# yjxiong/action-detection

Measured on AMD Instinct MI355X. Metric: proposals/sec (9-seg BNInception SSN fwd+bwd), higher is better.
Workload: dtype f32

## Files before the change

### action-detection_amd/_lib.py

```python
import ctypes
import os
import subprocess
import threading

import torch

_HERE = os.path.dirname(os.path.abspath(__file__))
CSRC = os.path.join(_HERE, "csrc")
LIB_PATH = os.path.join(_HERE, "libssn_hip.so")
SOURCES = ["conv_igemm.hip", "conv_x6.hip", "conv_x6_rect.hip", "conv_wgrad.hip", "conv_wgrad_x6.hip", "elementwise.hip", "bn_train.hip", "frames.hip", "detect.hip", "pool.hip", "stpp.hip", "heads_losses.hip", "conv_pl.hip", "planes_ops.hip", "planes_bn.hip", "wgrad_pl.hip", "tag.hip", "eval.hip", "actionness.hip", "train_step.hip"]

STPP_MAX_PARTS = 24


class SsnStppTable(ctypes.Structure):
    _fields_ = [("n_parts", ctypes.c_int), ("n_seg", ctypes.c_int),
                ("act_lo", ctypes.c_int), ("act_hi", ctypes.c_int),
                ("lo", ctypes.c_int * STPP_MAX_PARTS), ("hi", ctypes.c_int * STPP_MAX_PARTS),
                ("norm", ctypes.c_int * STPP_MAX_PARTS), ("col", ctypes.c_int * STPP_MAX_PARTS)]


_SIGS = {
    "ssn_conv_bn_relu_fwd": "pppppiiiiliiiliiiiipp",
    "ssn_bn_fold": "pppppfppip",
    "ssn_relu_bn_bwd": "pppiiillpp",
    "ssn_conv_dgrad": "pppiiiiliiiliiiiplpiipp",
    "ssn_conv_pack_weights": "ppiiiip",
    "ssn_conv_pack_weights_multi": "ippppppppp",
    "ssn_conv_wgrad": "ppppiiiiliiiliiiplip",
    "ssn_conv_wgrad_x6": "ppppiiiililiiiplippiipp",
    "ssn_wgrad_reduce": "pppiiip",
    "ssn_wgrad_reduce_taps": "pppiiiip",
    "ssn_conv_x6_pack_weights_multi": "ippppppppppppp",
    "ssn_conv_x6_fwd": "pppppiiiiliiiliiiiiippiiipp",
    "ssn_conv_x6_dgrad": "pppiiiiliiiliiiplpiippiipp",
    "ssn_conv_x6_fwd_rect": "pppppiiiiliiiliiiiiiippp",
    "ssn_conv_x6_pack_dgrad_s2": "ppiip",
    "ssn_conv_x6_dgrad_s2": "pppiiiiliiiliplpiippip",
    "ssn_conv_x6_pack_dgrad_rect": "ppiiiip",
    "ssn_conv_x6_pack_rect_multi": "ipppppppp",
    "ssn_conv_x6_dgrad_rect": "pppiiiililiiiiiplpiippp",
    "ssn_conv_wgrad_x6_rect": "ppppiiiililiiiiiplippp",
    "ssn_conv_x6_pack_weights_rect": "ppiiiip",
    "ssn_pool_fwd": "ipppiiiiliiliiipp",
    "ssn_pool_bwd": "ipppiiiiliiliiiiplppp",
    "ssn_avgpool_affine_fwd": "ppppiiiiiliiliiipp",
    "ssn_channel_sum": "ppiiilpup",
    "ssn_tensor_amax": "plpp",
    "ssn_bn_train_stats": "ppppppiiilffpup",
    "ssn_bn_train_apply": "ppppppiiiillpp",
    "ssn_bn_train_bwd": "pppppppppiiiillllpupp",
    "ssn_global_avgpool_fwd": "ppiiilp",
    "ssn_global_avgpool_bwd": "ppiiilipp",
    "ssn_dropout_fwd": "ppplfupp",
    "ssn_dropout_bwd": "ppplfp",
    "ssn_stpp_fwd": "ppppiipp",
    "ssn_stpp_bwd": "ppppiipp",
    "ssn_heads_fwd": "pppppppppppiipp",
    "ssn_heads_bwd": "pppppppppppiippppp",
    "ssn_stpp_reorg": "piippppiiiiipppp",
    "ssn_crop_mean": "ppiiip",
    "ssn_detections": "ppppppppuiiiiidip",
    "ssn_tag_count": "pppiipidppppp",
    "ssn_tag_generate": "ppppiipipippllddppppppppup",
    "ssn_tag_name_proposals": "pppippiidpppp",
    "ssn_eval_count": "ppiipp",
    "ssn_eval_ap": "ppppippiippiippllpppplp",
    "ssn_eval_recall": "ppippiipipp",
    "ssn_actionness_fc": "ppppiiiiiip",
    "ssn_actionness_group": "pppiiiip",
    "ssn_actionness_merge": "pppppiiiiip",
    "ssn_frames_crop_normalize": "ppiiiiiiipppiipipip",
    "ssn_frames_crop_resize_normalize": "ppiiiiiippiipipipup",
    "ssn_reg_denorm": "plffffp",
    "ssn_frame_diff": "ppliiip",
    "ssn_linear_fwd": "ppppiiip",
    "ssn_linear_bwd": "ppppppiiiip",
    "ssn_row_gather": "pppiip",
    "ssn_row_scatter": "pppiiip",
    "ssn_ce_loss_fwd": "ppppiip",
    "ssn_ce_loss_bwd": "pppppiip",
    "ssn_completeness_loss_fwd": "pppppiiiiiifp",
    "ssn_completeness_loss_bwd": "ppppiifp",
    "ssn_cw_smoothl1_fwd": "pppppiip",
    "ssn_total_loss_fwd": "ppiippiiiiiifpppiiffpppppp",
    "ssn_total_loss_bwd": "ppiipiifpiiffpppppppp",
    "ssn_label_select": "pppipipippppp",
    "ssn_param_checksum": "pipppip",
    "ssn_cw_smoothl1_bwd": "ppppiip",
    "ssn_sgd_step": "ppplffffipp",
    "ssn_sgd_step_multi": "ippppppffipp",
    "ssn_bn_fold_multi": "ipppppppppp",
    "ssn_sumsq": "plpipp",
# ... 54 lines not shown
        self.cdll.ssn_abi_version.restype = ctypes.c_int
        self.cdll.ssn_conv_wgrad_workspace_bytes.restype = ctypes.c_long
        self.cdll.ssn_conv_wgrad_workspace_bytes.argtypes = [ctypes.c_int] * 7
        self.cdll.ssn_conv_packed_floats.restype = ctypes.c_long
        self.cdll.ssn_conv_packed_floats.argtypes = [ctypes.c_int] * 4
        self.cdll.ssn_conv_x6_packed_floats.restype = ctypes.c_long
        self.cdll.ssn_conv_x6_packed_floats.argtypes = [ctypes.c_int] * 4
        self.cdll.ssn_conv_x6_dgrad_s2_packed_floats.restype = ctypes.c_long
        self.cdll.ssn_conv_x6_dgrad_s2_packed_floats.argtypes = [ctypes.c_int] * 2
        self.cdll.ssn_conv_x6_packed_floats_rect.restype = ctypes.c_long
        self.cdll.ssn_conv_x6_packed_floats_rect.argtypes = [ctypes.c_int] * 4
        self.cdll.ssn_conv_x6_packed_floats_dgrad_rect.restype = ctypes.c_long
        self.cdll.ssn_conv_x6_packed_floats_dgrad_rect.argtypes = [ctypes.c_int] * 4
        self.cdll.ssn_conv_wgrad_x6_rect_workspace_bytes.restype = ctypes.c_long
        self.cdll.ssn_conv_wgrad_x6_rect_workspace_bytes.argtypes = [ctypes.c_int] * 8
        self.cdll.ssn_conv_wgrad_x6_workspace_bytes.restype = ctypes.c_long
        self.cdll.ssn_conv_wgrad_x6_workspace_bytes.argtypes = [ctypes.c_int] * 7
        self.cdll.ssn_detections_workspace_bytes.restype = ctypes.c_size_t
        self.cdll.ssn_detections_workspace_bytes.argtypes = [ctypes.c_int] * 2
        self.cdll.ssn_tag_workspace_bytes.restype = ctypes.c_size_t
        self.cdll.ssn_tag_workspace_bytes.argtypes = [ctypes.c_long] * 2
        self.cdll.ssn_tag_lds_candidates.restype = ctypes.c_int
        self.cdll.ssn_tag_lds_candidates.argtypes = []
        self.cdll.ssn_eval_workspace_bytes.restype = ctypes.c_size_t
        self.cdll.ssn_eval_workspace_bytes.argtypes = [ctypes.c_long, ctypes.c_long, ctypes.c_int]
        self.cdll.ssn_eval_lds_gt.restype = ctypes.c_int
        self.cdll.ssn_eval_lds_gt.argtypes = []
        self.cdll.ssn_sumsq_multi_workspace_floats.restype = ctypes.c_long
        self.cdll.ssn_sumsq_multi_workspace_floats.argtypes = [ctypes.c_int, ctypes.c_void_p]
        self.cdll.ssn_train_step_launches.restype = ctypes.c_long
        self.cdll.ssn_train_step_launches.argtypes = [ctypes.c_int]
        self.cdll.ssn_conv_pick_tile.restype = ctypes.c_int
        self.cdll.ssn_conv_pick_tile.argtypes = [ctypes.c_int, ctypes.c_long]
        self.cdll.ssn_pl_channel_sum_workspace_bytes.restype = ctypes.c_long
        self.cdll.ssn_pl_channel_sum_workspace_bytes.argtypes = [ctypes.c_int]
        self.cdll.ssn_conv_x6_pack_entry_bytes.restype = ctypes.c_long
        self.cdll.ssn_conv_x6_pack_batch_abort.restype = None
        self.cdll.ssn_pl_bn_train_workspace_bytes.restype = ctypes.c_long
        self.cdll.ssn_pl_bn_train_workspace_bytes.argtypes = [ctypes.c_int]
        self.cdll.ssn_frames_resize_workspace_bytes.restype = ctypes.c_size_t
        self.cdll.ssn_frames_resize_workspace_bytes.argtypes = [ctypes.c_int] * 3
        self.cdll.ssn_conv_wgrad_pl_workspace_bytes.restype = ctypes.c_long
        self.cdll.ssn_conv_wgrad_pl_workspace_bytes.argtypes = [ctypes.c_int] * 8
        self.cdll.ssn_conv_wgrad_pl_group_workspace_bytes.restype = ctypes.c_long
        self.cdll.ssn_conv_wgrad_pl_group_workspace_bytes.argtypes = [ctypes.c_int, ctypes.c_void_p, ctypes.c_void_p, ctypes.c_void_p]
        self.cdll.ssn_conv_wgrad_pl_group_table_bytes.restype = ctypes.c_long
        self.cdll.ssn_conv_wgrad_pl_group_table_bytes.argtypes = [ctypes.c_int]
        self.cdll.ssn_conv_wgrad_pl_group_tuning.restype = None
        self.cdll.ssn_conv_wgrad_pl_group_tuning.argtypes = [ctypes.c_double, ctypes.c_double, ctypes.c_int, ctypes.c_int]
        self._fn = {}
        for name, sig in _SIGS.items():
            fn = getattr(self.cdll, name)
            fn.restype = ctypes.c_int
            fn.argtypes = [_CT[c] for c in sig]
            self._fn[name] = fn

    def call(self, name, *args):
        rc = self._fn[name](*args)
        if rc != 0:
            raise RuntimeError("%s failed (%d): %s" % (name, rc, self.cdll.ssn_last_error().decode()))

    def wgrad_workspace_bytes(self, n, cin, cout, ho, wo, ksize, tile_cfg=-1):
        return int(self.cdll.ssn_conv_wgrad_workspace_bytes(n, cin, cout, ho, wo, ksize, tile_cfg))


_lock = threading.Lock()
_lib = None
_test_lib = None


def _source_stamp(deps, flags):
    import hashlib
    h = hashlib.sha256(" ".join(flags).encode())
    for d in deps:
        h.update(os.path.basename(d).encode())
        with open(d, "rb") as f:
            h.update(f.read())
    return h.hexdigest()


def build(force=False, verbose=False):
    import fcntl
    srcs = [os.path.join(CSRC, s) for s in SOURCES]
    deps = srcs + [os.path.join(CSRC, h) for h in ("ssn_common.h", "conv_epilogue.h", "conv_x6_kernel.h", "planes.h", "conv_pl_epilogue.inc")]
    flags = ["--offload-arch=gfx950", "-O3", "-std=c++17", "-fPIC"]
    stamp_path = LIB_PATH + ".stamp"
    want = _source_stamp(deps, flags)

    def fresh():
        if not os.path.exists(LIB_PATH) or not os.path.exists(stamp_path):
            return False
        with open(stamp_path) as f:
            return f.read().strip() == want

    if not force and fresh():
        return LIB_PATH
    with open(LIB_PATH + ".lock", "w") as lock:
        fcntl.flock(lock, fcntl.LOCK_EX)
        try:
            if not force and fresh():
                return LIB_PATH
            hipcc = os.environ.get("HIPCC", "/opt/rocm/bin/hipcc")
            objs = []
            procs = []
            headers = deps[len(srcs):]
            for s in srcs:
                o = os.path.join(CSRC, os.path.basename(s) + ".o")
                objs.append(o)
                ostamp = _source_stamp([s] + headers, flags)
                try:
                    with open(o + ".stamp") as f:
                        if not force and os.path.exists(o) and f.read().strip() == ostamp:
                            continue
                except OSError:
                    pass
                cmd = [hipcc] + flags + ["-c", s, "-o", o]
                procs.append((cmd, o, ostamp, subprocess.Popen(cmd, stdout=subprocess.PIPE, stderr=subprocess.STDOUT)))
            for cmd, o, ostamp, p in procs:
                out, _ = p.communicate()
                if verbose and out:
                    print(out.decode())
                if p.returncode != 0:
                    raise RuntimeError("hipcc failed: %s\n%s" % (" ".join(cmd), out.decode()))
                with open(o + ".stamp", "w") as f:
                    f.write(ostamp + "\n")
            tmp = LIB_PATH + ".tmp.%d" % os.getpid()
            subprocess.check_call([hipcc, "--offload-arch=gfx950", "-shared", "-fPIC", "-o", tmp] + objs)
            os.replace(tmp, LIB_PATH)
            with open(stamp_path, "w") as f:
                f.write(want + "\n")
        finally:
            fcntl.flock(lock, fcntl.LOCK_UN)
    return LIB_PATH


def get_lib():
    global _lib
    if _test_lib is not None:
        return _test_lib
    if _lib is None:
        with _lock:
            if _lib is None:
                if not os.path.exists(LIB_PATH):
                    raise RuntimeError(
                        "libssn_hip.so is missing (%s). Build it with __graft_entry__.build() / "
                        "action_detection_amd.build(); there is no CPU fallback." % LIB_PATH)
                _lib = SsnLibrary(LIB_PATH)
    return _lib


def use_library_for_testing(lib):
    global _test_lib
    _test_lib = lib


def emulator_active():
    return _test_lib is not None and _test_lib.is_emulator
```

### action-detection_amd/csrc/conv_pl.hip

```cpp
#include "planes.h"

namespace {

using namespace pl;

enum { MODE_FWD = 0, MODE_DGRAD = 1 };

constexpr int APITCH = 16;

struct PlConvArgs {
    const void* x_hi;
    const void* x_lo;
    const uint32_t* ap;
    const float* x_scale;
    const float* y_scale;
    float* y_amax;
    void* y_hi;
    void* y_lo;
    const float* scale;
    const float* shift;
    int N, C, H, W;
    uint32_t x_img_bytes;
    uint32_t x_grp_bytes;
    int M;
    int Ho, Wo;
    uint32_t y_img_bytes, y_grp_bytes;
    int P;
    int kh, kw, stride, pad_h, pad_w;
    int relu, accumulate;
    int raw_from;
    int row_split, row_gap;
    int k_split, k_gap;
    const void* mask_hi;
    const float* mask_scale;
    uint32_t mask_img_bytes;
    int n_ptiles, n_mtiles, ngroups;
    uint32_t x_bytes, a_bytes, y_bytes, mask_bytes;
    int sub_a, sub_b, sub_W;
    uint32_t magic_wp;
    FastDiv div_sp;
    unsigned long long* trace;
    int dbg;
    FastDiv div_hw, div_w, div_mt;
    FastDiv div_tpi;
};

#ifdef PL_ABLATE
#define PL_DBG(bit) (p.dbg & (bit))
#else
#define PL_DBG(bit) 0
#endif

#if defined(__HIP_DEVICE_COMPILE__)
#define PL_DMA_B128(rsrc_, dst_, voff_, soff_) \
    __builtin_amdgcn_raw_ptr_buffer_load_lds(rsrc_, SSN_LDS_PTR(dst_), 16, voff_, soff_, 0, 0)
#else
#define PL_DMA_B128(rsrc_, dst_, voff_, soff_) ((void)(dst_), (void)(voff_), (void)(soff_))
#endif

template <int MODE, int WM, int WN, int TM, int TN>
__global__ __launch_bounds__(256, (TM * TN >= 8) ? 1 : 2) void conv_pl_kernel(PlConvArgs p) {
    constexpr int NW = 4;
    constexpr int NT = 256;
    constexpr int BM = WM * TM * 32;
    constexpr int BN = WN * TN * 32;
    static_assert(WM * WN == 4, "4 waves");
    static_assert(BN % 64 == 0 && BN <= 256, "tile width 64 / 128 / 256 pixels");
    constexpr int SEGS = BN / 64;
    constexpr int A_PIECES = BM / 16;
    constexpr int NA = (A_PIECES + NW - 1) / NW;
    constexpr int A_STAGE = NA * NW * 256;
    constexpr int PK = BN * 4;
    constexpr int B_STAGE = 4 * PK;
    constexpr int STAGE = A_STAGE + B_STAGE;
    constexpr bool ONE_WAVE = (TM * TN >= 8);
    constexpr int NSTAGE = (STAGE * 4 * 4 * (ONE_WAVE ? 1 : 2) <= 163840) ? 4 : 3;
    constexpr int NB = 4 * SEGS / NW;
    constexpr int NLOAD = NA + NB;

    __shared__ __attribute__((aligned(1024))) uint32_t lds[NSTAGE * STAGE];

    const int tid = threadIdx.x;
    const int lane = tid & 63, wave = wave_uniform(tid >> 6);
    const int wm = wave / WN, wn = wave % WN;
    const int li = lane & 31, lh = lane >> 5;

    const uint32_t nblk = (uint32_t)p.n_ptiles * (uint32_t)p.n_mtiles;
    const uint32_t logical = xcd_remap(blockIdx.x, nblk);
    uint32_t ptile, mtile;
    fd_divmod(logical, p.div_mt, ptile, mtile);
    const int m0 = (int)mtile * BM;
    const int p0 = (int)ptile * BN;
    const int KK = p.kh * p.kw;
    unsigned long long tr0 = 0, tr1 = 0, tr2 = 0, trr = 0;
    if (p.trace) {
        tr0 = __builtin_readcyclecounter();
        trr = __builtin_amdgcn_s_memrealtime();
    }

    const int seg = wave % SEGS;
    uint32_t gbase;
    uint32_t gmask = 0;
    {
        const int gp = p0 + seg * 64 + lane;
        const bool gvalid = gp < p.P;
        uint32_t n, hw, ho, wo;
        fd_divmod((uint32_t)(gvalid ? gp : 0), p.div_hw, n, hw);
        fd_divmod(hw, p.div_w, ho, wo);
        const int h0 = (MODE == MODE_FWD) ? (int)ho * p.stride - p.pad_h : (int)ho + p.pad_h;
        const int w0 = (MODE == MODE_FWD) ? (int)wo * p.stride - p.pad_w : (int)wo + p.pad_w;
        int t = 0;
        for (int r = 0; r < p.kh; ++r)
            for (int s = 0; s < p.kw; ++s, ++t) {
                const int hi = (MODE == MODE_FWD) ? h0 + r : h0 - r;
                const int wi = (MODE == MODE_FWD) ? w0 + s : w0 - s;
                if (gvalid && ((unsigned)hi < (unsigned)p.H) && ((unsigned)wi < (unsigned)p.W)) gmask |= 1u << t;
            }
        gbase = n * p.x_img_bytes + (uint32_t)((h0 * p.W + w0) * 16);
        if (PL_DBG(1)) gmask = 0;
    }

    uint32_t aoff[NA];
#pragma unroll
    for (int q = 0; q < NA; ++q) {
        const int f = (q * NW + wave) * 64 + lane;
        aoff[q] = (f < BM * 4 && m0 + f / 4 < p.M && !PL_DBG(2)) ? (uint32_t)(m0 * APITCH) * 4u + (uint32_t)f * 16u : PL_OOB;
    }
    const __amdgpu_buffer_rsrc_t xrsrc[2] = {pl_rsrc(p.x_hi, p.x_bytes), pl_rsrc(p.x_lo, p.x_bytes)};
    const __amdgpu_buffer_rsrc_t arsrc = pl_rsrc(p.ap, p.a_bytes);
    const uint32_t a_step = (uint32_t)(p.M * APITCH) * 4u;
    const int nslab = p.ngroups * KK;
    const bool c_half = (p.C & 8) != 0;

    int pf_g = 0, pf_tap = 0, pf_col = 0;
// ... 359 lines not shown
        __builtin_amdgcn_s_barrier();
        __builtin_amdgcn_sched_barrier(0);
        const int ntap = tap == 8 ? 0 : tap + 1, nhb = tap == 8 ? hb ^ 1 : hb;
        const uint32_t dead = (tap + NSTAGE >= 9) ? tail_dead : 0u;
        auto piece = [&](int k) {
            if (k == 0)
                issue_halo(nx_live, nx_so, hb ^ 1, tap);
            else
                issue_a(s_cur, dead, k - 1);
        };
#pragma unroll
        for (int c = 0; c < 3; ++c)
#pragma unroll
            for (int i = 0; i < TM; ++i)
#pragma unroll
                for (int j = 0; j < TN; ++j) {
                    acc[i][j] = __builtin_amdgcn_mfma_f32_32x32x16_f16(f.af[PA[c]][i], f.bf[PB[c]][j], acc[i][j], 0, 0, 0);
                    const int idx = (c * TM + i) * TN + j;
#pragma unroll
                    for (int k = idx * NREAD / NM; k < (idx + 1) * NREAD / NM; ++k)
                        if (!PL_DBG(4)) read_step(nxt, k, s_n1, nhb, ntap);
                    if ((idx + 1) % EVERY == 0 && (idx + 1) / EVERY <= NLOAD) piece((idx + 1) / EVERY - 1);
                    __builtin_amdgcn_sched_barrier(0);
                }
#pragma unroll
        for (int k = NM / EVERY; k < NLOAD; ++k) piece(k);
        pf_a += a_step;
        const uint32_t o = s_cur;
        s_cur = s_n1;
        s_n1 = s_n2;
        if (NSTAGE == 4) {
            s_n2 = s_n3;
            s_n3 = o;
        } else {
            s_n2 = o;
        }
    };
    auto group = [&](int g, Frags& fa, Frags& fb, int hb) {
        group_begin(g);
#pragma unroll
        for (int tap = 0; tap < 9; ++tap) {
            if (tap & 1)
                slab(fb, fa, tap, hb);
            else
                slab(fa, fb, tap, hb);
        }
    };
    int g = 0;
    for (; g + 1 < p.ngroups; g += 2) {
        group(g, fr0, fr1, 0);
        group(g + 1, fr1, fr0, 1);
    }
    if (g < p.ngroups) group(g, fr0, fr1, 0);
    SSN_WAIT_LGKM0();
    SSN_WAIT_VMCNT(0);

#define PL_PEND (PI ? pl_pend : p.P)
#include "conv_pl_epilogue.inc"
#undef PL_PEND
}
#undef PL_DMA_B128

int g_pl_default_tile = -1;
int g_pl_dbg = 0;
unsigned long long* g_pl_trace = nullptr;

template <int MODE, int WM, int WN, int TM, int TN>
int launch_cfg(PlConvArgs& a, hipStream_t stream) {
    constexpr int BM = WM * TM * 32;
    constexpr int BN = WN * TN * 32;
    a.n_mtiles = (a.M + BM - 1) / BM;
    a.div_mt = make_fastdiv((uint32_t)a.n_mtiles);
    a.n_ptiles = (a.P + BN - 1) / BN;
    const unsigned nblk = (unsigned)a.n_ptiles * (unsigned)a.n_mtiles;
    hipLaunchKernelGGL((conv_pl_kernel<MODE, WM, WN, TM, TN>), dim3(nblk), dim3(256), 0, stream, a);
    SSN_CHECK_LAUNCH("conv_pl");
    return SSN_OK;
}

constexpr int PL_NCFG = 12;
const int kPlBM[PL_NCFG] = {128, 64, 128, 64, 192, 256, 128, 96, 160, 32, 64, 192};
const int kPlBN[PL_NCFG] = {128, 128, 64, 64, 128, 128, 256, 128, 128, 128, 256, 64};

template <int MODE>
int launch_tile(PlConvArgs& a, int cfg, hipStream_t stream) {
    switch (cfg) {
        case 0: return launch_cfg<MODE, 2, 2, 2, 2>(a, stream);
        case 1: return launch_cfg<MODE, 2, 2, 1, 2>(a, stream);
        case 2: return launch_cfg<MODE, 2, 2, 2, 1>(a, stream);
        case 3: return launch_cfg<MODE, 2, 2, 1, 1>(a, stream);
        case 4: return launch_cfg<MODE, 2, 2, 3, 2>(a, stream);
        case 5: return launch_cfg<MODE, 2, 2, 4, 2>(a, stream);
        case 6: return launch_cfg<MODE, 2, 2, 2, 4>(a, stream);
        case 7: return launch_cfg<MODE, 1, 4, 3, 1>(a, stream);
        case 8: return launch_cfg<MODE, 1, 4, 5, 1>(a, stream);
        case 9: return launch_cfg<MODE, 1, 4, 1, 1>(a, stream);
        case 10: return launch_cfg<MODE, 2, 2, 1, 4>(a, stream);
        case 11: return launch_cfg<MODE, 2, 2, 3, 1>(a, stream);
    }
    ssn_set_error("conv_pl: unknown tile config %d", cfg);
    return SSN_ERR_ARG;
}

template <int MODE, int WM, int WN, int TM, int TN, bool PI = false>
int launch_cfg9(PlConvArgs& a, hipStream_t stream) {
    constexpr int BM = WM * TM * 32;
    constexpr int BN = WN * TN * 32;
    a.n_mtiles = (a.M + BM - 1) / BM;
    a.div_mt = make_fastdiv((uint32_t)a.n_mtiles);
    if (PI) {
        const int tpi = (a.H * a.W + BN - 1) / BN;
        a.div_tpi = make_fastdiv((uint32_t)tpi);
        a.n_ptiles = a.N * tpi;
    } else {
        a.div_tpi = make_fastdiv(1u);
        a.n_ptiles = (a.P + BN - 1) / BN;
    }
    const unsigned nblk = (unsigned)a.n_ptiles * (unsigned)a.n_mtiles;
    hipLaunchKernelGGL((conv_pl9_kernel<MODE, WM, WN, TM, TN, PI>), dim3(nblk), dim3(256), 0, stream, a);
    SSN_CHECK_LAUNCH("conv_pl9");
    return SSN_OK;
}
bool halo_tile_pi(int cfg) { return cfg == 0 || cfg == 1 || cfg == 4 || cfg == 7 || cfg == 8 || cfg == 9; }
template <int MODE>
int launch_tile9_pi(PlConvArgs& a, int cfg, hipStream_t stream) {
    switch (cfg) {
        case 0: return launch_cfg9<MODE, 2, 2, 2, 2, true>(a, stream);
        case 1: return launch_cfg9<MODE, 2, 2, 1, 2, true>(a, stream);
        case 4: return launch_cfg9<MODE, 2, 2, 3, 2, true>(a, stream);
        case 7: return launch_cfg9<MODE, 1, 4, 3, 1, true>(a, stream);
        case 8: return launch_cfg9<MODE, 1, 4, 5, 1, true>(a, stream);
        case 9: return launch_cfg9<MODE, 1, 4, 1, 1, true>(a, stream);
    }
    ssn_set_error("conv_pl9: tile config %d has no per-image haloed variant", cfg);
    return SSN_ERR_ARG;
}
bool halo_fits_pi(int H, int W, int bn, int hs) {
    const int Wp = W + 2;
    auto slot = [&](int q) { return (q / W + 1) * Wp + (q % W) + 1; };
    for (int p0 = 0; p0 < H * W; p0 += bn) {
        const int p1 = p0 + bn - 1 < H * W - 1 ? p0 + bn - 1 : H * W - 1;
        if (slot(p1) - slot(p0) + 2 * (Wp + 1) + 1 > hs) return false;
    }
    return true;
}
bool halo_tile(int cfg) { return cfg == 0 || cfg == 1 || cfg == 2 || cfg == 3 || cfg == 4 || cfg == 7 || cfg == 8 || cfg == 9 || cfg == 11; }
template <int MODE>
int launch_tile9(PlConvArgs& a, int cfg, hipStream_t stream) {
    switch (cfg) {
        case 0: return launch_cfg9<MODE, 2, 2, 2, 2>(a, stream);
        case 1: return launch_cfg9<MODE, 2, 2, 1, 2>(a, stream);
        case 2: return launch_cfg9<MODE, 2, 2, 2, 1>(a, stream);
        case 3: return launch_cfg9<MODE, 2, 2, 1, 1>(a, stream);
        case 4: return launch_cfg9<MODE, 2, 2, 3, 2>(a, stream);
        case 7: return launch_cfg9<MODE, 1, 4, 3, 1>(a, stream);
        case 8: return launch_cfg9<MODE, 1, 4, 5, 1>(a, stream);
        case 9: return launch_cfg9<MODE, 1, 4, 1, 1>(a, stream);
        case 11: return launch_cfg9<MODE, 2, 2, 3, 1>(a, stream);
    }
    ssn_set_error("conv_pl9: tile config %d has no haloed variant", cfg);
    return SSN_ERR_ARG;
}
bool halo_fits(int N, int H, int W, int bn, int hs) {
    const long P = (long)N * H * W;
    const int Wp = W + 2, SP = (H + 2) * Wp;
    auto slot = [&](long pp) { return (pp / (H * W)) * SP + ((pp % (H * W)) / W + 1) * Wp + (pp % W) + 1; };
    for (long t = 0; t * bn < P; ++t) {
        const long p0 = t * bn, p1 = (p0 + bn - 1 < P - 1) ? p0 + bn - 1 : P - 1;
// ... 19 lines not shown
    }
    if (cfg >= PL_HALO_BASE) {
        cfg -= PL_HALO_BASE;
        if (halo_layer && cfg < PL_NCFG && halo_tile(cfg) && halo_fits(a.N, a.H, a.W, kPlBN[cfg], kPlBN[cfg] == 128 ? 320 : 192)) {
            a.magic_wp = (uint32_t)((0x100000000ull + (unsigned)(a.W + 2) - 1) / (unsigned)(a.W + 2));
            a.div_sp = make_fastdiv((uint32_t)((a.H + 2) * (a.W + 2)));
            return launch_tile9<MODE>(a, cfg, stream);
        }
    }
    return launch_tile<MODE>(a, cfg, stream);
}

int default_tile(int M, long P) {
    double best = 1e300;
    int bc = 0;
    for (int c = 0; c < PL_NCFG; ++c) {
        if (c == 5 || c == 6 || c == 10) continue;
        const long mt = (M + kPlBM[c] - 1) / kPlBM[c], pt = (P + kPlBN[c] - 1) / kPlBN[c];
        const double padded = (double)(mt * kPlBM[c]) * (double)(pt * kPlBN[c]);
        const double small = (kPlBM[c] * kPlBN[c] >= 128 * 128) ? 1.0 : (kPlBM[c] * kPlBN[c] >= 64 * 128 ? 1.1 : 1.3);
        const long blocks = mt * pt;
        const double fill = blocks < 256 ? 256.0 / (double)blocks : 1.0;
        const double cost = padded * small * fill;
        if (cost < best) {
            best = cost;
            bc = c;
        }
    }
    return bc;
}

int fill_common(PlConvArgs& a, const void* x_hi, const void* x_lo, const uint32_t* ap, void* y_hi, void* y_lo, int N, int C,
                int H, int W, long x_img_groups, int M, int Ho, int Wo, long y_img_groups, int kh, int kw,
                const float* x_scale, const float* y_scale, float* y_amax, int k_gap, int row_gap, const char* what) {
    SSN_CHECK_ARG(x_hi && x_lo && ap && y_hi && y_lo && x_scale && y_scale, "%s: null pointer", what);
    SSN_CHECK_ARG(C > 0 && C % 8 == 0 && M > 0 && M % 8 == 0, "%s: channel counts must be multiples of 8 (C %d, M %d)", what, C, M);
    SSN_CHECK_ARG(kh >= 1 && kw >= 1 && kh * kw <= 32, "%s: %dx%d taps unsupported", what, kh, kw);
    a.x_hi = x_hi;
    a.x_lo = x_lo;
    a.ap = ap;
    a.y_hi = y_hi;
    a.y_lo = y_lo;
    a.x_scale = x_scale;
    a.y_scale = y_scale;
    a.y_amax = y_amax;
    a.N = N;
    a.C = C;
    a.H = H;
    a.W = W;
    a.M = M;
    a.Ho = Ho;
    a.Wo = Wo;
    a.kh = kh;
    a.kw = kw;
    a.P = N * Ho * Wo;
    a.ngroups = (C + 15) / 16;
    const long xg = (long)H * W * 16, yg = (long)Ho * Wo * 16;
    const long xb = (long)N * x_img_groups * xg, yb = (long)N * y_img_groups * yg;
    const long ab = (long)a.ngroups * kh * kw * M * APITCH * 4;
    SSN_CHECK_ARG(x_img_groups >= (C + k_gap) / 8 && y_img_groups >= (M + row_gap) / 8, "%s: slice wider than its tensor", what);
    SSN_CHECK_ARG(xb < (1l << 31) && yb < (1l << 31) && ab < (1l << 31) && (long)N * Ho * Wo < (1l << 31),
                  "%s: operand plane larger than 2 GiB (buffer addressing)", what);
    a.x_grp_bytes = (uint32_t)xg;
    a.y_grp_bytes = (uint32_t)yg;
    a.x_img_bytes = (uint32_t)(x_img_groups * xg);
    a.y_img_bytes = (uint32_t)(y_img_groups * yg);
    a.x_bytes = (uint32_t)((long)(N - 1) * a.x_img_bytes + (long)((C + k_gap) / 8) * xg);
    a.y_bytes = (uint32_t)((long)(N - 1) * a.y_img_bytes + (long)((M + row_gap) / 8) * yg);
    a.a_bytes = (uint32_t)ab;
    a.div_hw = make_fastdiv((uint32_t)(Ho * Wo));
    a.div_w = make_fastdiv((uint32_t)Wo);
    a.sub_a = a.sub_b = a.sub_W = 0;
    a.mask_hi = nullptr;
    a.mask_scale = nullptr;
    a.mask_img_bytes = 0;
    a.mask_bytes = 0;
    a.k_split = 0;
    a.k_gap = 0;
    a.row_split = 0x7fffffff;
    a.row_gap = 0;
    a.raw_from = 0x7fffffff;
    a.scale = a.shift = nullptr;
    a.relu = a.accumulate = 0;
    a.dbg = g_pl_dbg;
    a.trace = g_pl_trace;
    return SSN_OK;
}

}

extern "C" int ssn_conv_pl_tiles(void) { return PL_NCFG; }
extern "C" int ssn_conv_pl_halo_taken(int N, int H, int W, int tile_cfg) {
    if (tile_cfg >= PL_HALO_PI_BASE) {
        const int c = tile_cfg - PL_HALO_PI_BASE;
        return c < PL_NCFG && halo_tile_pi(c) && halo_fits_pi(H, W, 128, 320);
    }
    const int cfg = tile_cfg - PL_HALO_BASE;
    return cfg >= 0 && cfg < PL_NCFG && halo_tile(cfg) && halo_fits(N, H, W, kPlBN[cfg], kPlBN[cfg] == 128 ? 320 : 192);
}
extern "C" void ssn_conv_pl_debug_flags(int flags) { g_pl_dbg = flags; }
extern "C" void ssn_conv_pl_debug_trace(unsigned long long* buf) { g_pl_trace = buf; }
extern "C" int ssn_conv_pl_tile_shape(int cfg, int* bm, int* bn) {
    if (cfg < 0 || cfg >= PL_NCFG) return SSN_ERR_ARG;
    *bm = kPlBM[cfg];
    *bn = kPlBN[cfg];
    return SSN_OK;
}

extern "C" int ssn_conv_pl_fwd(const void* x_hi, const void* x_lo, const float* w_packed, const float* scale,
                               const float* shift, void* y_hi, void* y_lo, int N, int Cin, int H, int W,
                               long x_img_groups, int Cout, int Ho, int Wo, long y_img_groups, int kh, int kw, int stride,
                               int pad_h, int pad_w, int relu, int tile_cfg, const float* x_scale, const float* y_scale,
                               float* y_amax, int raw_from, int row_split, int row_gap, hipStream_t stream) {
    PlConvArgs a;
    int rc = fill_common(a, x_hi, x_lo, (const uint32_t*)w_packed, y_hi, y_lo, N, Cin, H, W, x_img_groups, Cout, Ho, Wo,
                         y_img_groups, kh, kw, x_scale, y_scale, y_amax, 0, row_gap, "conv pl fwd");
    if (rc != SSN_OK) return rc;
    SSN_CHECK_ARG(stride == 1 || stride == 2, "conv pl fwd: stride %d unsupported", stride);
    SSN_CHECK_ARG(!row_gap || (row_split % 32 == 0 && row_gap % 8 == 0 && row_split > 0 && row_split < Cout),
                  "conv pl fwd: a row split must be a multiple of 32 inside (0, M), the gap a multiple of 8");
    a.stride = stride;
    a.pad_h = pad_h;
    a.pad_w = pad_w;
    a.scale = scale;
    a.shift = shift;
    a.relu = relu;
    a.raw_from = raw_from > 0 ? raw_from : 0x7fffffff;
    if (row_gap) {
        a.row_split = row_split;
        a.row_gap = row_gap;
    }
    const int cfg = tile_cfg >= 0 ? tile_cfg : (g_pl_default_tile >= 0 ? g_pl_default_tile : default_tile(Cout, a.P));
    const bool halo_layer = kh == 3 && kw == 3 && stride == 1 && pad_h == 1 && pad_w == 1 && Ho == H && Wo == W && !row_gap;
    return launch_any<MODE_FWD>(a, cfg, halo_layer, stream);
}

extern "C" int ssn_conv_pl_dgrad(const void* dy_hi, const void* dy_lo, const float* wt_packed, void* dx_hi, void* dx_lo,
                                 int N, int Cout, int Ho, int Wo, long dy_img_groups, int Cin, int H, int W,
                                 long dx_img_groups, int kh, int kw, int pad_h, int pad_w, int accumulate,
                                 const void* mask_hi, long mask_img_groups, const float* mask_scale, int tile_cfg,
                                 const float* dy_scale, const float* dx_scale, float* dx_amax, int k_split, int k_gap,
                                 int taps_reversed, hipStream_t stream) {
    PlConvArgs a;
    int rc = fill_common(a, dy_hi, dy_lo, (const uint32_t*)wt_packed, dx_hi, dx_lo, N, Cout, Ho, Wo, dy_img_groups, Cin, H, W,
                         dx_img_groups, kh, kw, dy_scale, dx_scale, dx_amax, k_gap, 0, "conv pl dgrad");
    if (rc != SSN_OK) return rc;
    SSN_CHECK_ARG(!k_gap || (k_split % 16 == 0 && k_gap % 8 == 0 && k_split > 0 && k_split < Cout && Cout % 16 == 0),
                  "conv pl dgrad: a channel split must be a multiple of 16 inside (0, C)");
    a.stride = 1;
    a.pad_h = pad_h;
    a.pad_w = pad_w;
    a.accumulate = accumulate;
    a.k_split = k_split;
    a.k_gap = k_gap;
    if (mask_hi && mask_scale) {
        a.mask_hi = mask_hi;
        a.mask_scale = mask_scale;
        const long mg = (long)H * W * 16;
        SSN_CHECK_ARG(mask_img_groups >= Cin / 8 && (long)N * mask_img_groups * mg < (1l << 31), "conv pl dgrad: bad mask tensor");
        a.mask_img_bytes = (uint32_t)(mask_img_groups * mg);
        a.mask_bytes = (uint32_t)((long)(N - 1) * a.mask_img_bytes + (long)(Cin / 8) * mg);
    }
    const int cfg = tile_cfg >= 0 ? tile_cfg : (g_pl_default_tile >= 0 ? g_pl_default_tile : default_tile(Cin, a.P));
    if (taps_reversed) {
        a.pad_h = kh - 1 - pad_h;
        a.pad_w = kw - 1 - pad_w;
        return launch_tile<MODE_FWD>(a, plain_tile(cfg), stream);
// ... 50 lines not shown
```

Before: 2307.

## Add specialized one-tap conv kernel for 1x1 stride-1 planes convolutions

```diff
diff --git a/action-detection_amd/_lib.py b/action-detection_amd/_lib.py
--- a/action-detection_amd/_lib.py
+++ b/action-detection_amd/_lib.py
@@ -8,7 +8,7 @@
 _HERE = os.path.dirname(os.path.abspath(__file__))
 CSRC = os.path.join(_HERE, "csrc")
 LIB_PATH = os.path.join(_HERE, "libssn_hip.so")
-SOURCES = ["conv_igemm.hip", "conv_x6.hip", "conv_x6_rect.hip", "conv_wgrad.hip", "conv_wgrad_x6.hip", "elementwise.hip", "bn_train.hip", "frames.hip", "detect.hip", "pool.hip", "stpp.hip", "heads_losses.hip", "conv_pl.hip", "planes_ops.hip", "planes_bn.hip", "wgrad_pl.hip", "tag.hip", "eval.hip", "actionness.hip", "train_step.hip"]
+SOURCES = ["conv_igemm.hip", "conv_x6.hip", "conv_x6_rect.hip", "conv_wgrad.hip", "conv_wgrad_x6.hip", "elementwise.hip", "bn_train.hip", "frames.hip", "detect.hip", "pool.hip", "stpp.hip", "heads_losses.hip", "conv_pl.hip", "conv_pl1.hip", "planes_ops.hip", "planes_bn.hip", "wgrad_pl.hip", "tag.hip", "eval.hip", "actionness.hip", "train_step.hip"]
 
 STPP_MAX_PARTS = 24
 
@@ -229,7 +229,7 @@
 def build(force=False, verbose=False):
     import fcntl
     srcs = [os.path.join(CSRC, s) for s in SOURCES]
-    deps = srcs + [os.path.join(CSRC, h) for h in ("ssn_common.h", "conv_epilogue.h", "conv_x6_kernel.h", "planes.h", "conv_pl_epilogue.inc")]
+    deps = srcs + [os.path.join(CSRC, h) for h in ("ssn_common.h", "conv_epilogue.h", "conv_x6_kernel.h", "planes.h", "conv_pl_epilogue.inc", "conv_pl_args.h")]
     flags = ["--offload-arch=gfx950", "-O3", "-std=c++17", "-fPIC"]
     stamp_path = LIB_PATH + ".stamp"
     want = _source_stamp(deps, flags)
diff --git a/action-detection_amd/csrc/conv_pl.hip b/action-detection_amd/csrc/conv_pl.hip
--- a/action-detection_amd/csrc/conv_pl.hip
+++ b/action-detection_amd/csrc/conv_pl.hip
@@ -1,55 +1,12 @@
-#include "planes.h"
+#include <cstdlib>
+
+#include "conv_pl_args.h"
 
 namespace {
 
 using namespace pl;
 
 enum { MODE_FWD = 0, MODE_DGRAD = 1 };
-
-constexpr int APITCH = 16;
-
-struct PlConvArgs {
-    const void* x_hi;
-    const void* x_lo;
-    const uint32_t* ap;
-    const float* x_scale;
-    const float* y_scale;
-    float* y_amax;
-    void* y_hi;
-    void* y_lo;
-    const float* scale;
-    const float* shift;
-    int N, C, H, W;
-    uint32_t x_img_bytes;
-    uint32_t x_grp_bytes;
-    int M;
-    int Ho, Wo;
-    uint32_t y_img_bytes, y_grp_bytes;
-    int P;
-    int kh, kw, stride, pad_h, pad_w;
-    int relu, accumulate;
-    int raw_from;
-    int row_split, row_gap;
-    int k_split, k_gap;
-    const void* mask_hi;
-    const float* mask_scale;
-    uint32_t mask_img_bytes;
-    int n_ptiles, n_mtiles, ngroups;
-    uint32_t x_bytes, a_bytes, y_bytes, mask_bytes;
-    int sub_a, sub_b, sub_W;
-    uint32_t magic_wp;
-    FastDiv div_sp;
-    unsigned long long* trace;
-    int dbg;
-    FastDiv div_hw, div_w, div_mt;
-    FastDiv div_tpi;
-};
-
-#ifdef PL_ABLATE
-#define PL_DBG(bit) (p.dbg & (bit))
-#else
-#define PL_DBG(bit) 0
-#endif
 
 #if defined(__HIP_DEVICE_COMPILE__)
 #define PL_DMA_B128(rsrc_, dst_, voff_, soff_) \
@@ -575,8 +532,20 @@
 const int kPlBM[PL_NCFG] = {128, 64, 128, 64, 192, 256, 128, 96, 160, 32, 64, 192};
 const int kPlBN[PL_NCFG] = {128, 128, 64, 64, 128, 128, 256, 128, 128, 128, 256, 64};
 
+bool one_tap_enabled() {
+    static const bool env_on = [] {
+        const char* e = getenv("SSN_PL_ONE_TAP");
+        return !(e && e[0] == '0' && e[1] == 0);
+    }();
+    return env_on && !(g_pl_dbg & PL_FLAG_NO_ONE_TAP);
+}
+bool one_tap_layer(const PlConvArgs& a) {
+    return a.kh == 1 && a.kw == 1 && a.stride == 1 && a.pad_h == 0 && a.pad_w == 0 && a.Ho == a.H && a.Wo == a.W && a.sub_W == 0;
+}
+
 template <int MODE>
 int launch_tile(PlConvArgs& a, int cfg, hipStream_t stream) {
+    if (one_tap_layer(a) && pl1_has_tile(cfg) && one_tap_enabled()) return pl1_launch(a, cfg, stream);
     switch (cfg) {
         case 0: return launch_cfg<MODE, 2, 2, 2, 2>(a, stream);
         case 1: return launch_cfg<MODE, 2, 2, 1, 2>(a, stream);
@@ -762,7 +731,7 @@
     a.raw_from = 0x7fffffff;
     a.scale = a.shift = nullptr;
     a.relu = a.accumulate = 0;
-    a.dbg = g_pl_dbg;
+    a.dbg = g_pl_dbg & ~PL_FLAG_NO_ONE_TAP;
     a.trace = g_pl_trace;
     return SSN_OK;
 }
diff --git a/action-detection_amd/csrc/conv_pl1.hip b/action-detection_amd/csrc/conv_pl1.hip
--- /dev/null
+++ b/action-detection_amd/csrc/conv_pl1.hip
@@ -0,0 +1,272 @@
+#include "conv_pl_args.h"
+
+namespace {
+
+using namespace pl;
+
+#if defined(__HIP_DEVICE_COMPILE__)
+#define PL1_DMA_B128(rsrc_, dst_, voff_, soff_) \
+    __builtin_amdgcn_raw_ptr_buffer_load_lds(rsrc_, SSN_LDS_PTR(dst_), 16, voff_, soff_, 0, 0)
+#else
+#define PL1_DMA_B128(rsrc_, dst_, voff_, soff_) ((void)(dst_), (void)(voff_), (void)(soff_))
+#endif
+#if defined(__AMDGCN__)
+#define PL1_PIN_SGPR(x) asm volatile("" : "+s"(x))
+#else
+#define PL1_PIN_SGPR(x) ((void)0)
+#endif
+
+template <int WM, int WN, int TM, int TN>
+__global__ __launch_bounds__(256, (TM * TN >= 8) ? 1 : 2) void conv_pl1_kernel(PlConvArgs p) {
+    constexpr int NW = 4;
+    constexpr int NT = 256;
+    constexpr int BM = WM * TM * 32;
+    constexpr int BN = WN * TN * 32;
+    static_assert(WM * WN == 4, "4 waves");
+    static_assert(BN % 64 == 0 && BN <= 256, "tile width 64 / 128 / 256 pixels");
+    constexpr int SEGS = BN / 64;
+    constexpr int A_PIECES = BM / 16;
+    constexpr int NA = (A_PIECES + NW - 1) / NW;
+    constexpr int A_STAGE = NA * NW * 256;
+    constexpr int PK = BN * 4;
+    constexpr int B_STAGE = 4 * PK;
+    constexpr int STAGE = A_STAGE + B_STAGE;
+    constexpr int NSTAGE = 4;
+    static_assert(STAGE * 4 * NSTAGE * ((TM * TN >= 8) ? 1 : 2) <= 163840, "the ring of every co-resident workgroup fits the 160 KiB of LDS");
+    constexpr int NB = 4 * SEGS / NW;
+    constexpr int NLOAD = NA + NB;
+
+    __shared__ __attribute__((aligned(1024))) uint32_t lds[NSTAGE * STAGE];
+
+    const int tid = threadIdx.x;
+    const int lane = tid & 63, wave = wave_uniform(tid >> 6);
+    const int wm = wave / WN, wn = wave % WN;
+    const int li = lane & 31, lh = lane >> 5;
+
+    const uint32_t nblk = (uint32_t)p.n_ptiles * (uint32_t)p.n_mtiles;
+    const uint32_t logical = xcd_remap(blockIdx.x, nblk);
+    uint32_t ptile, mtile;
+    fd_divmod(logical, p.div_mt, ptile, mtile);
+    const int m0 = (int)mtile * BM;
+    const int p0 = (int)ptile * BN;
+
+    const int seg = wave % SEGS;
+    uint32_t bvo[NB];
+    __amdgpu_buffer_rsrc_t brsrc[NB];
+    int bdst[NB];
+    bool bhalf[NB];
+    {
+        const int gp = p0 + seg * 64 + lane;
+        const bool gvalid = gp < p.P && !PL_DBG(1);
+        uint32_t n, hw;
+        fd_divmod((uint32_t)(gvalid ? gp : 0), p.div_hw, n, hw);
+        const uint32_t vo = n * p.x_img_bytes + hw * 16u;
+#pragma unroll
+        for (int k = 0; k < NB; ++k) {
+            const int pk = (wave + k * NW) / SEGS;
+            bhalf[k] = (pk & 1) != 0;
+            bvo[k] = gvalid ? vo + (bhalf[k] ? p.x_grp_bytes : 0u) : PL_OOB;
+            brsrc[k] = pl_rsrc((pk >> 1) ? p.x_lo : p.x_hi, p.x_bytes);
+            bdst[k] = A_STAGE + seg * 256 + pk * PK;
+        }
+    }
+
+    uint32_t aoff[NA];
+#pragma unroll
+    for (int q = 0; q < NA; ++q) {
+        const int f = (q * NW + wave) * 64 + lane;
+        aoff[q] = (f < BM * 4 && m0 + f / 4 < p.M && !PL_DBG(2)) ? (uint32_t)(m0 * APITCH) * 4u + (uint32_t)f * 16u : PL_OOB;
+    }
+    const __amdgpu_buffer_rsrc_t arsrc = pl_rsrc(p.ap, p.a_bytes);
+    const uint32_t a_step = (uint32_t)(p.M * APITCH) * 4u;
+    const int nslab = p.ngroups;
+    const bool c_half = (p.C & 8) != 0;
+
+    int pf_g = 0;
+    uint32_t pf_x = 0, pf_a = 0;
+    const uint32_t group_step = 2u * p.x_grp_bytes;
+    const uint32_t gap_at = p.k_gap ? (uint32_t)(p.k_split / 16) * group_step : 0xffffffffu;
+    const uint32_t gap_to = gap_at + (uint32_t)(p.k_gap / 8) * p.x_grp_bytes;
+    uint32_t d_so, d_aso, d_dead;
+    bool d_tail;
+    auto issue_begin = [&](bool fast) {
+        d_so = pf_x;
+        d_aso = pf_a;
+        if (!fast) {
+            d_dead = pf_g >= nslab ? PL_OOB : 0u;
+            d_tail = (pf_g == nslab - 1) && c_half;
+            ++pf_g;
+        }
+        pf_a += a_step;
+        PL1_PIN_SGPR(pf_a);
+        pf_x += group_step;
+        pf_x = (pf_x == gap_at) ? gap_to : pf_x;
+    };
+    auto issue_piece = [&](int k, uint32_t st_off, bool fast) {
+        if (k < NB) {
+            uint32_t v = bvo[k];
+            if (!fast) {
+                if (d_tail && bhalf[k]) v = PL_OOB;
+                v |= d_dead;
+            }
+            PL1_DMA_B128(brsrc[k], lds + st_off + bdst[k], v, d_so);
+        } else {
+            const int q = k - NB;
+            PL1_DMA_B128(arsrc, lds + st_off + wave * 256 + q * NW * 256, fast ? aoff[q] : (aoff[q] | d_dead), d_aso);
+        }
+    };
+
+    f32x16 acc[TM][TN];
+#pragma unroll
+    for (int i = 0; i < TM; ++i)
+#pragma unroll
+        for (int j = 0; j < TN; ++j)
+#pragma unroll
+            for (int r = 0; r < 16; ++r) acc[i][j][r] = 0.f;
+
+#pragma unroll
+    for (int st = 0; st < NSTAGE; ++st) {
+        issue_begin(false);
+#pragma unroll
+        for (int k = 0; k < NLOAD; ++k) issue_piece(k, st * STAGE, false);
+    }
+
+    const float sa = f16_scale_of(__builtin_bit_cast(float, p.ap[p.a_bytes >> 2]));
+    const float sb = *p.x_scale;
+    const float so = *p.y_scale;
+    const float inv = so / (sa * sb);
+    float ep_mul = inv, ep_add = 0.f, ep_msc = __builtin_nanf(""), ep_flo = -__builtin_inff();
+    if (tid < BM) {
+        const int m = m0 + tid;
+        const bool ok = m < p.M;
+        const bool aff = ok && p.scale && m < p.raw_from;
+        if (aff) {
+            ep_mul = p.scale[m + (m >= p.row_split ? p.row_gap : 0)] * inv;
+            ep_add = p.shift[m] * so;
+        }
+        if (ok && p.mask_scale) ep_msc = p.mask_scale[m];
+        if (p.relu && m < p.raw_from) ep_flo = 0.f;
+    }
+
+    const int swz = (li >> 2) & 3;
+    int achunk[2];
+#pragma unroll
+    for (int pn = 0; pn < 2; ++pn) achunk[pn] = ((2 * pn + lh) ^ swz) * 4;
+    const int arow = (wm * TM * 32 + li) * APITCH;
+    const int bcol = A_STAGE + lh * PK + (wn * TN * 32 + li) * 4;
+
+    struct Frags {
+        f16x8 af[2][TM];
+        f16x8 bf[2][TN];
+    };
+    Frags fr0, fr1;
+    constexpr int NREAD = 2 * TN + 2 * TM;
+    auto read_step = [&](Frags& f, int k, uint32_t st_off) {
+        if (k < 2 * TN) {
+            const int pn = k / TN, j = k % TN;
+            f.bf[pn][j] = __builtin_bit_cast(f16x8, *reinterpret_cast<const u32x4*>(lds + st_off + bcol + pn * 2 * PK + j * 128));
+        } else {
+            const int q = k - 2 * TN, pn = q / TM, i = q % TM;
+            f.af[pn][i] = __builtin_bit_cast(f16x8, *reinterpret_cast<const u32x4*>(lds + st_off + arow + i * 32 * APITCH + achunk[pn]));
+        }
+    };
+    auto slab = [&](const Frags& f, Frags& nxt, uint32_t dma_off, uint32_t rd_off, bool fast) {
+        constexpr int PA[3] = {1, 0, 0};
+        constexpr int PB[3] = {0, 0, 1};
+        constexpr int NM = 3 * TM * TN;
+        constexpr int EVERY = NM / NLOAD > 0 ? NM / NLOAD : 1;
+        SSN_WAIT_VMCNT((NSTAGE - 2) * NLOAD);
+        SSN_WAIT_LGKM0();
+        __builtin_amdgcn_s_barrier();
+        __builtin_amdgcn_sched_barrier(0);
+        issue_begin(fast);
+        __builtin_amdgcn_sched_barrier(0);
+#pragma unroll
+        for (int c = 0; c < 3; ++c)
+#pragma unroll
+            for (int i = 0; i < TM; ++i)
+#pragma unroll
+                for (int j = 0; j < TN; ++j) {
+                    acc[i][j] = __builtin_amdgcn_mfma_f32_32x32x16_f16(f.af[PA[c]][i], f.bf[PB[c]][j], acc[i][j], 0, 0, 0);
+                    const int idx = (c * TM + i) * TN + j;
+#pragma unroll
+                    for (int k = idx * NREAD / NM; k < (idx + 1) * NREAD / NM; ++k)
+                        if (!PL_DBG(4)) read_step(nxt, k, rd_off);
+                    if ((idx + 1) % EVERY == 0 && (idx + 1) / EVERY <= NLOAD) issue_piece((idx + 1) / EVERY - 1, dma_off, fast);
+                    __builtin_amdgcn_sched_barrier(0);
+                }
+#pragma unroll
+        for (int k = NM / EVERY; k < NLOAD; ++k) issue_piece(k, dma_off, fast);
+    };
+
+    SSN_WAIT_VMCNT((NSTAGE - 1) * NLOAD);
+    __builtin_amdgcn_s_barrier();
+#pragma unroll
+    for (int k = 0; k < NREAD; ++k) read_step(fr0, k, 0u);
+
+    const int nfull = nslab - (c_half ? 1 : 0);
+    int t = 0;
+    for (; t + 2 * NSTAGE <= nfull; t += NSTAGE) {
+        slab(fr0, fr1, 0 * STAGE, 1 * STAGE, true);
+        slab(fr1, fr0, 1 * STAGE, 2 * STAGE, true);
+        slab(fr0, fr1, 2 * STAGE, 3 * STAGE, true);
+        slab(fr1, fr0, 3 * STAGE, 0 * STAGE, true);
+    }
+    pf_g = t + NSTAGE;
+    uint32_t s_cur = 0, s_n1 = STAGE, s_n2 = 2 * STAGE, s_n3 = 3 * STAGE;
+    auto rotate = [&]() {
+        const uint32_t o = s_cur;
+        s_cur = s_n1;
+        s_n1 = s_n2;
+        s_n2 = s_n3;
+        s_n3 = o;
+    };
+    for (; t < nslab; t += 2) {
+        slab(fr0, fr1, s_cur, s_n1, false);
+        rotate();
+        slab(fr1, fr0, s_cur, s_n1, false);
+        rotate();
+    }
+    SSN_WAIT_LGKM0();
+    SSN_WAIT_VMCNT(0);
+
+#define PL_PEND p.P
+#include "conv_pl_epilogue.inc"
+#undef PL_PEND
+}
+#undef PL1_DMA_B128
+#undef PL1_PIN_SGPR
+
+template <int WM, int WN, int TM, int TN>
+int launch_cfg1(PlConvArgs& a, hipStream_t stream) {
+    constexpr int BM = WM * TM * 32;
+    constexpr int BN = WN * TN * 32;
+    a.n_mtiles = (a.M + BM - 1) / BM;
+    a.div_mt = make_fastdiv((uint32_t)a.n_mtiles);
+    a.n_ptiles = (a.P + BN - 1) / BN;
+    const unsigned nblk = (unsigned)a.n_ptiles * (unsigned)a.n_mtiles;
+    hipLaunchKernelGGL((conv_pl1_kernel<WM, WN, TM, TN>), dim3(nblk), dim3(256), 0, stream, a);
+    SSN_CHECK_LAUNCH("conv_pl1");
+    return SSN_OK;
+}
+
+}
+
+bool pl::pl1_has_tile(int cfg) { return cfg >= 0 && cfg < 12 && cfg != 5 && cfg != 6; }
+
+int pl::pl1_launch(PlConvArgs& a, int cfg, hipStream_t stream) {
+    switch (cfg) {
+        case 0: return launch_cfg1<2, 2, 2, 2>(a, stream);
+        case 1: return launch_cfg1<2, 2, 1, 2>(a, stream);
+        case 2: return launch_cfg1<2, 2, 2, 1>(a, stream);
+        case 3: return launch_cfg1<2, 2, 1, 1>(a, stream);
+        case 4: return launch_cfg1<2, 2, 3, 2>(a, stream);
+        case 7: return launch_cfg1<1, 4, 3, 1>(a, stream);
+        case 8: return launch_cfg1<1, 4, 5, 1>(a, stream);
+        case 9: return launch_cfg1<1, 4, 1, 1>(a, stream);
+        case 10: return launch_cfg1<2, 2, 1, 4>(a, stream);
+        case 11: return launch_cfg1<2, 2, 3, 1>(a, stream);
+    }
+    ssn_set_error("conv_pl1: tile config %d has no one-tap variant", cfg);
+    return SSN_ERR_ARG;
+}
diff --git a/action-detection_amd/csrc/conv_pl_args.h b/action-detection_amd/csrc/conv_pl_args.h
--- /dev/null
+++ b/action-detection_amd/csrc/conv_pl_args.h
@@ -0,0 +1,56 @@
+#pragma once
+#include "planes.h"
+
+namespace pl {
+
+constexpr int APITCH = 16;
+
+struct PlConvArgs {
+    const void* x_hi;
+    const void* x_lo;
+    const uint32_t* ap;
+    const float* x_scale;
+    const float* y_scale;
+    float* y_amax;
+    void* y_hi;
+    void* y_lo;
+    const float* scale;
+    const float* shift;
+    int N, C, H, W;
+    uint32_t x_img_bytes;
+    uint32_t x_grp_bytes;
+    int M;
+    int Ho, Wo;
+    uint32_t y_img_bytes, y_grp_bytes;
+    int P;
+    int kh, kw, stride, pad_h, pad_w;
+    int relu, accumulate;
+    int raw_from;
+    int row_split, row_gap;
+    int k_split, k_gap;
+    const void* mask_hi;
+    const float* mask_scale;
+    uint32_t mask_img_bytes;
+    int n_ptiles, n_mtiles, ngroups;
+    uint32_t x_bytes, a_bytes, y_bytes, mask_bytes;
+    int sub_a, sub_b, sub_W;
+    uint32_t magic_wp;
+    FastDiv div_sp;
+    unsigned long long* trace;
+    int dbg;
+    FastDiv div_hw, div_w, div_mt;
+    FastDiv div_tpi;
+};
+
+#ifdef PL_ABLATE
+#define PL_DBG(bit) (p.dbg & (bit))
+#else
+#define PL_DBG(bit) 0
+#endif
+
+constexpr int PL_FLAG_NO_ONE_TAP = 1 << 16;
+
+bool pl1_has_tile(int cfg);
+int pl1_launch(PlConvArgs& a, int cfg, hipStream_t stream);
+
+}
```

Measured after the change: 2320, median of 6. No clear change (+0.5%).
